# PolarisRisingWar/rgb-experiment

Measured on AMD Instinct MI355X. Metric: aggregated edges/sec (full-graph GCN d=128, reference epoch = train fwd+bwd+Adam + 2 eval fwd), higher is better.
Workload: dtype f32

## Files before the change

include/rgbx_hip.h:

```cpp
#ifndef RGBX_HIP_H
#define RGBX_HIP_H

#include <stddef.h>
#include <stdint.h>

#ifdef __cplusplus
extern "C" {
#endif

#define RGBX_VERSION 501

#define RGBX_OK 0
#define RGBX_E_ARG (-1)
#define RGBX_E_RANGE (-2)
#define RGBX_E_ALIGN (-3)
#define RGBX_E_WS (-4)
#define RGBX_E_SHAPE (-5)

typedef void* rgbx_stream_t;

enum {
  RGBX_LOOPS_KEEP = 0,
  RGBX_LOOPS_ADD_REMAINING = 1,
  RGBX_LOOPS_REMOVE_ADD = 2
// ... 230 lines not shown
int rgbx_masked_nll_bwd_f32(const int64_t* y, const uint8_t* mask, int64_t N, int64_t C,
                            const float* scale, float* grad, int64_t ldg, rgbx_stream_t stream);

int rgbx_masked_ce_fwd_f32(const float* logits, int64_t ld, const int64_t* y, const uint8_t* mask, int64_t N,
                           int64_t C, double* stats, double* scratch, int64_t scratch_doubles,
                           rgbx_stream_t stream);

int rgbx_masked_ce_fwd_blocked_f32(const float* logits, int64_t blk_cols, int64_t blk_stride, const float* bias,
                                   const int64_t* y, const uint8_t* mask, int64_t N, int64_t C, double* stats,
                                   double* scratch, int64_t scratch_doubles, rgbx_stream_t stream);

int rgbx_masked_ce_bwd_f32(const float* logits, int64_t ld, const int64_t* y, const uint8_t* mask, int64_t N,
                           int64_t C, const float* scale, float* grad, int64_t ldg, rgbx_stream_t stream);


int rgbx_coalesce_workspace_bytes(int64_t E, int64_t N, int mirror, size_t* bytes);
int rgbx_coalesce_keys_i64(const int64_t* row, const int64_t* col, int64_t E, int64_t N, int mirror,
                           uint64_t* keys_out, uint64_t* counts, void* workspace, size_t workspace_bytes,
                           rgbx_stream_t stream);
int rgbx_split_edge_keys_i64(const uint64_t* keys, const uint64_t* counts, int64_t cap, int64_t N, int64_t* out_row,
                             int64_t* out_col, rgbx_stream_t stream);

int rgbx_py_random_shuffle_i64(int64_t seed, int64_t n, int64_t* perm);


int rgbx_gather_rows_f32(const float* src, int64_t lds, const int32_t* idx, int64_t n, int64_t d,
                         float* dst, int64_t ldd, rgbx_stream_t stream);

int rgbx_scatter_add_rows_f32(const float* src, int64_t lds, const int32_t* idx, int64_t n,
                              int64_t d, float* dst, int64_t ldd, rgbx_stream_t stream);

int rgbx_paced_copy_f32(const float* src, float* dst, int64_t n, int workgroups, int nontemporal, rgbx_stream_t stream);

#ifdef __cplusplus
}
#endif
#endif
```

rgb_experiment_amd/_lib.py:

```python
import ctypes
import os

import torch

_HERE = os.path.dirname(os.path.abspath(__file__))
LIB_PATH = os.path.join(_HERE, "csrc", "librgbx_hip.so")

_P = ctypes.c_void_p
_I64 = ctypes.c_int64
_I = ctypes.c_int
_F = ctypes.c_float

class RowSplit(ctypes.Structure):
    _fields_ = [("threshold", ctypes.c_int32), ("n_chunks", ctypes.c_int32), ("n_long", ctypes.c_int32),
                ("chunk_begin", ctypes.c_void_p), ("chunk_end", ctypes.c_void_p), ("chunk_row", ctypes.c_void_p),
                ("long_row", ctypes.c_void_p),
                ("long_chunk_ptr", ctypes.c_void_p), ("partial", ctypes.c_void_p)]


class CeEpilogue(ctypes.Structure):
    _fields_ = [("y", ctypes.c_void_p), ("mask", ctypes.c_void_p), ("grad_scale", ctypes.c_void_p),
                ("stats", ctypes.c_void_p), ("scratch", ctypes.c_void_p), ("mask_groups", ctypes.c_int32),
                ("rows", ctypes.c_void_p), ("n_rows", ctypes.c_int64), ("skip_unselected", ctypes.c_int32)]

# ... 21 lines not shown
    "rgbx_inv_degree_f32": [_P, _I64, _P, _P],
    "rgbx_spmm_csr_f32": [_P, _P, _P, _P, _P, _I64, _P, _I64, _P, _P, _I64, _I64, _I64, _F, _F, _P, _P],
    "rgbx_spmm_csr_epilogue_supported": [_I64],
    "rgbx_spmm_csr_epilogue_f32": [_P, _P, _P, _P, _P, _I64, _P, _I64, _P, _P, _I64, _I64, _I64, _F, _F, _P, _P, _P],
    "rgbx_spmm_csr_short_rows_supported": [_I64],
    "rgbx_spmm_csr_short_rows_f32": [_P, _P, _P, _P, _I64, _P, _P, _I64, _I64, _I64, _P],
    "rgbx_spmm_linear_supported": [_I64, _I64, _I],
    "rgbx_spmm_linear_stats_workspace_bytes": [_I64, _I64, ctypes.POINTER(ctypes.c_size_t)],
    "rgbx_spmm_linear_f32": [_P, _P, _P, _P, _P, _I64, _P, _P, _I64, _P, _P, _P, _I64, _P, _I64, _P, _P, _P, _P, _P,
                             ctypes.c_size_t, _P, _I64, _I64, _I64, _P, _P],
    "rgbx_fused_layer_f32": [_P, _P],
    "rgbx_blocked_to_rows_f32": [_P, _I64, _I64, _P, _I64, _I64, _I64, _P, _P],
    "rgbx_appnp_f32": [_P, _P, _P, _P, _I64, _P, _P, _I64, _I64, _I64, _I, _F, _P, _P],
    "rgbx_dagnn_gate_fwd_f32": [_P, _I64, _P, _I64, _I64, _P, _P, _P, _I64, _I64, _I64, _I, _P],
    "rgbx_dagnn_gate_bwd_workspace_bytes": [_I64, ctypes.POINTER(ctypes.c_size_t)],
    "rgbx_dagnn_gate_bwd_f32": [_P, _I64, _P, _I64, _I64, _P, _P, _P, _I64, _P, _I64, _P, _I64, _I64, _P, _P, _P,
                                ctypes.c_size_t, _I64, _I64, _I, _P],
    "rgbx_gru_step_supported": [_I64],
    "rgbx_gru_step_f32": [_P, _P, _P, _I64, _P, _P, _P, _P, _I64, _P, _I64, _P, _I64, _I64, _I64, _P, _P],
    "rgbx_gru_gate_fwd_f32": [_P, _I64, _P, _I64, _P, _I64, _I64, _I64, _P],
    "rgbx_gru_gate_bwd_f32": [_P, _I64, _P, _I64, _P, _I64, _P, _I64, _P, _I64, _I64, _I64, _P],
    "rgbx_gat_scores_f32": [_P, _I64, _P, _P, _P, _P, _I64, _I, _I, _P],
    "rgbx_gat_scores_bwd_scratch_floats": [_I64, _I, _I, ctypes.POINTER(ctypes.c_int64)],
    "rgbx_gat_scores_bwd_f32": [_P, _I64, _P, _P, _I64, _P, _P, _P, _I64, _P, _P, _P, _I64, _I64, _I, _I, _P],
    "rgbx_gat_aggregate_fwd_f32": [_P, _P, _P, _I64, _P, _P, _P, _P, _P, _P, _P, _I64, _P, _P, _P, _P, _I64, _I, _I, _F, _P,
                                   _P],
    "rgbx_gat_edge_softmax_f32": [_P, _P, _P, _P, _F, _P, _P, _P, _P, _P, _I64, _P, _P],
    "rgbx_gat_bwd_dst_f32": [_P, _P, _P, _I64, _P, _P, _P, _P, _P, _I64, _P, _I64, _P, _P, _I64, _I, _I,
                             _F, _P],
    "rgbx_gat_bwd_prep_f32": [_P, _P, _P, _P, _I64, _P, _P, _I64, _P, _P, _P, _F, _P, _I64, _I, _I, _P],
    "rgbx_gat_bwd_src_f32": [_P, _P, _P, _I64, _P, _P, _P, _I64, _P, _I64, _P, _P, _P, _P, _I64, _I, _I, _F, _P, _P],
    "rgbx_gemm_tn_workspace_bytes": [_I64, _I64, _I64, ctypes.POINTER(ctypes.c_size_t)],
    "rgbx_gemm_tn_f32": [_P, _I64, _P, _I64, _P, _I64, _P, _I64, _I64, _I64, _F, _P, ctypes.c_size_t, _P],
    "rgbx_bn_scratch_doubles": [_I64, _I64, ctypes.POINTER(ctypes.c_int64)],
    "rgbx_bn_stats_f32": [_P, _I64, _I64, _I64, _P, _P, _I64, _P],
    "rgbx_bn_finalize_f32": [_P, _P, _P, _F, _F, _P, _P, _P, _P, _P, _P, _I64, _P],
    "rgbx_fold_bn_linear_f32": [_P, _I64, _P, _I64, _P, _P, _P, _P, _P, _P, _F, _P, _P, _P, _I64, _I64, _P],
    "rgbx_bn_bwd_finalize_f32": [_P, _P, _P, _P, _P, _P, _P, _P, _P, _P, _I64, _P],
    "rgbx_affine_cols_f32": [_P, _I64, _P, _P, _P, _I64, _I64, _I64, _P],
    "rgbx_bn_bwd_reduce_f32": [_P, _I64, _P, _I64, _P, _P, _I64, _I64, _P, _P, _I64, _P],
    "rgbx_bn_bwd_apply_f32": [_P, _I64, _P, _I64, _P, _P, _P, _P, _P, _P, _I64, _I64, _I64, _P],
    "rgbx_masked_nll_scratch_doubles": [_I64, _I, ctypes.POINTER(ctypes.c_int64)],
    "rgbx_masked_nll_fwd_f32": [_P, _I64, _P, _P, _I64, _I64, _P, _P, _I64, _I, _P],
    "rgbx_masked_ce_fwd_f32": [_P, _I64, _P, _P, _I64, _I64, _P, _P, _I64, _P],
    "rgbx_masked_ce_fwd_blocked_f32": [_P, _I64, _I64, _P, _P, _P, _I64, _I64, _P, _P, _I64, _P],
    "rgbx_masked_ce_bwd_f32": [_P, _I64, _P, _P, _I64, _I64, _P, _P, _I64, _P],
    "rgbx_masked_nll_bwd_f32": [_P, _P, _I64, _I64, _P, _P, _I64, _P],
    "rgbx_coalesce_workspace_bytes": [_I64, _I64, _I, ctypes.POINTER(ctypes.c_size_t)],
    "rgbx_coalesce_keys_i64": [_P, _P, _I64, _I64, _I, _P, _P, _P, ctypes.c_size_t, _P],
    "rgbx_split_edge_keys_i64": [_P, _P, _I64, _I64, _P, _P, _P],
    "rgbx_gather_rows_f32": [_P, _I64, _P, _I64, _I64, _P, _I64, _P],
    "rgbx_scatter_add_rows_f32": [_P, _I64, _P, _I64, _I64, _P, _I64, _P],
    "rgbx_paced_copy_f32": [_P, _P, _I64, _I, _I, _P],
    "rgbx_py_random_shuffle_i64": [_I64, _I64, _P],
}
EXPORTS = ["rgbx_version", "rgbx_last_error_string"] + list(SIGNATURES)

_lib = None


def bind(path, strict=True):
    lib = ctypes.CDLL(path)
    lib.rgbx_version.restype = _I
    lib.rgbx_version.argtypes = []
    lib.rgbx_last_error_string.restype = ctypes.c_char_p
    lib.rgbx_last_error_string.argtypes = []
# ... 57 lines not shown
```

rgb_experiment_amd/csrc/gemm.hip:

```cpp
#include "rgbx_common.h"

namespace rgbx {
namespace {

constexpr int BM = 128, BN = 128, KT = 32;
using f32x16 = __attribute__((ext_vector_type(16))) float;

template <int W>
__device__ __forceinline__ void stage_tile(float* __restrict__ lds, const float* __restrict__ src,
                                           int64_t ld, int64_t k0, int64_t k_end, int c0, int ncols) {
  const int tid = threadIdx.x;
#pragma unroll 4
  for (int p = 0; p < KT * W / 256; ++p) {
    const int idx = p * 256 + tid;
    const int r = idx / W, c = idx % W;
    const int64_t k = k0 + r;
    lds[r * W + c] = (k < k_end && c0 + c < ncols) ? src[k * ld + c0 + c] : 0.f;
  }
}

template <int W>
__device__ __forceinline__ void fetch_tile(float4 (&regs)[KT * (W / 4) / 256], const float* __restrict__ src, int64_t ld,
                                           int64_t k0, int64_t k_end, int c0, int ncols) {
#pragma unroll
  for (int p = 0; p < KT * (W / 4) / 256; ++p) {
    const int idx = p * 256 + threadIdx.x;
    const int r = idx / (W / 4), c = (idx % (W / 4)) * 4;
    const int64_t k = k0 + r;
    regs[p] = make_float4(0.f, 0.f, 0.f, 0.f);
    if (k < k_end && c0 + c < ncols) regs[p] = *reinterpret_cast<const float4*>(src + k * ld + c0 + c);
  }
}

template <int W>
__device__ __forceinline__ void put_tile(float* __restrict__ lds, const float4 (&regs)[KT * (W / 4) / 256]) {
#pragma unroll
  for (int p = 0; p < KT * (W / 4) / 256; ++p) {
    const int idx = p * 256 + threadIdx.x;
    const int r = idx / (W / 4), c = (idx % (W / 4)) * 4;
    *reinterpret_cast<float4*>(lds + r * W + c) = regs[p];
  }
}

template <bool VEC4, int MT>
__global__ void __launch_bounds__(256)
gemm_tn_partial_kernel(const float* __restrict__ A, int64_t lda, const float* __restrict__ B, int64_t ldb,
                       float* __restrict__ part, float* __restrict__ colpart, int64_t K, int M, int N,
                       int64_t slab) {
  constexpr int MI = MT / 64;
  __shared__ float lds[KT * (MT + 128)];
  float* la = lds;
  float* lb = lds + KT * MT;
  const int split = blockIdx.x;
  const int m0 = blockIdx.y * MT, n0 = blockIdx.z * BN;
  const int64_t k_begin = (int64_t)split * slab;
  const int64_t k_end = k_begin + slab < K ? k_begin + slab : K;
  const int wave = threadIdx.x >> 6, lane = threadIdx.x & 63;
  const int wm = (wave >> 1) * (MT / 2), wn = (wave & 1) * 64;
  const int kr = lane >> 5, cc = lane & 31;

  f32x16 acc[MI][2];
#pragma unroll
  for (int i = 0; i < MI; ++i)
#pragma unroll
    for (int j = 0; j < 2; ++j)
#pragma unroll
      for (int r = 0; r < 16; ++r) acc[i][j][r] = 0.f;

  const bool sums = colpart != nullptr && blockIdx.z == 0 && threadIdx.x < MT;
  float csum = 0.f;
  auto consume = [&]() {
    if (sums) {
#pragma unroll 8
      for (int r = 0; r < KT; ++r) csum += la[r * MT + threadIdx.x];
    }
#pragma unroll 4
    for (int kk = 0; kk < KT; kk += 2) {
      float a[MI];
#pragma unroll
      for (int i = 0; i < MI; ++i) a[i] = la[(kk + kr) * MT + wm + i * 32 + cc];
      const float b0 = lb[(kk + kr) * 128 + wn + cc];
      const float b1 = lb[(kk + kr) * 128 + wn + 32 + cc];
#pragma unroll
      for (int i = 0; i < MI; ++i) {
        acc[i][0] = __builtin_amdgcn_mfma_f32_32x32x2f32(a[i], b0, acc[i][0], 0, 0, 0);
        acc[i][1] = __builtin_amdgcn_mfma_f32_32x32x2f32(a[i], b1, acc[i][1], 0, 0, 0);
      }
    }
  };
  if constexpr (VEC4) {
    float4 ra[KT * (MT / 4) / 256], rb[KT * 32 / 256];
    fetch_tile<MT>(ra, A, lda, k_begin, k_end, m0, M);
    fetch_tile<128>(rb, B, ldb, k_begin, k_end, n0, N);
    for (int64_t k0 = k_begin; k0 < k_end; k0 += KT) {
      __syncthreads();
      put_tile<MT>(la, ra);
      put_tile<128>(lb, rb);
      __syncthreads();
      if (k0 + KT < k_end) {
        fetch_tile<MT>(ra, A, lda, k0 + KT, k_end, m0, M);
        fetch_tile<128>(rb, B, ldb, k0 + KT, k_end, n0, N);
      }
      consume();
    }
  } else {
    for (int64_t k0 = k_begin; k0 < k_end; k0 += KT) {
      __syncthreads();
      stage_tile<MT>(la, A, lda, k0, k_end, m0, M);
      stage_tile<128>(lb, B, ldb, k0, k_end, n0, N);
      __syncthreads();
      consume();
    }
  }

  if (sums && m0 + (int)threadIdx.x < M) colpart[(int64_t)split * M + m0 + threadIdx.x] = csum;
  float* out = part + (int64_t)split * M * N;
#pragma unroll
  for (int i = 0; i < MI; ++i)
#pragma unroll
    for (int j = 0; j < 2; ++j)
#pragma unroll
      for (int r = 0; r < 16; ++r) {
        const int m = m0 + wm + i * 32 + (r & 3) + 8 * (r >> 2) + 4 * kr;
        const int n = n0 + wn + j * 32 + cc;
        if (m < M && n < N) out[(int64_t)m * N + n] = acc[i][j][r];
      }
}

__global__ void __launch_bounds__(256)
gemm_tn_reduce_kernel(const float* __restrict__ part, int S, int64_t MN, float* __restrict__ C, int N,
                      int64_t ldc, float alpha) {
  __shared__ float sh[8][32];
  const int j = threadIdx.x & 31, q = threadIdx.x >> 5;
  for (int64_t base = (int64_t)blockIdx.x * 32; base < MN; base += (int64_t)gridDim.x * 32) {
    const int64_t i = base + j;
    float s = 0.f;
    if (i < MN)
      for (int p = q; p < S; p += 8) s += part[(int64_t)p * MN + i];
    __syncthreads();
    sh[q][j] = s;
    __syncthreads();
    if (q == 0 && i < MN) {
      float t = 0.f;
#pragma unroll
      for (int k = 0; k < 8; ++k) t += sh[k][j];
      C[(i / N) * ldc + (i % N)] = alpha * t;
    }
  }
}

int tile_rows(int M) { return M <= 64 ? 64 : BM; }

int choose_splits(int64_t K, int M, int N) {
  const int64_t tiles = cdiv(M, tile_rows(M)) * cdiv(N, BN);
  int64_t s = cdiv(tile_rows(M) == 64 ? 1024 : 768, tiles);
  const int64_t max_s = cdiv(K, 16 * KT);
  if (s > max_s) s = max_s;
  if (s < 1) s = 1;
  return (int)s;
}

}
}

using namespace rgbx;

extern "C" int rgbx_gemm_tn_workspace_bytes(int64_t K, int64_t M, int64_t N, size_t* bytes) {
  if (!bytes || K < 0 || M < 0 || N < 0) return fail(RGBX_E_ARG, "gemm_tn_workspace_bytes: bad argument");
  if (M >= INT32_MAX || N >= INT32_MAX) return fail(RGBX_E_RANGE, "gemm_tn: M or N exceeds int32");
  *bytes = (size_t)choose_splits(K, (int)M, (int)N) * ((size_t)M * (size_t)N + (size_t)M) * sizeof(float);
  return RGBX_OK;
}

extern "C" int rgbx_gemm_tn_f32(const float* A, int64_t lda, const float* B, int64_t ldb, float* C,
                                int64_t ldc, float* a_colsum, int64_t K, int64_t M, int64_t N, float alpha,
                                void* workspace, size_t workspace_bytes, rgbx_stream_t stream) {
  if (K < 0 || M < 0 || N < 0) return fail(RGBX_E_ARG, "gemm_tn: negative size");
  if (M == 0 || N == 0) return RGBX_OK;
  if (!C || (K > 0 && (!A || !B))) return fail(RGBX_E_ARG, "gemm_tn: null pointer");
  if (M >= INT32_MAX || N >= INT32_MAX) return fail(RGBX_E_RANGE, "gemm_tn: M or N exceeds int32");
  if (lda < M || ldb < N || ldc < N) return fail(RGBX_E_ARG, "gemm_tn: leading dimension too small");
  size_t need = 0;
  if (int rc = rgbx_gemm_tn_workspace_bytes(K, M, N, &need)) return rc;
  if (!workspace || workspace_bytes < need)
    return fail(RGBX_E_WS, "gemm_tn: workspace %zu < %zu bytes", workspace_bytes, need);
  hipStream_t s = (hipStream_t)stream;
  const int S = choose_splits(K, (int)M, (int)N);
  const int64_t slab = cdiv(cdiv(K > 0 ? K : 1, S), KT) * KT;
  float* part = static_cast<float*>(workspace);
  float* colpart = a_colsum ? part + (size_t)S * M * N : nullptr;
  const int mt = tile_rows((int)M);
  dim3 grid(S, (unsigned)cdiv(M, mt), (unsigned)cdiv(N, BN));
  const bool v4 = aligned16(A) && aligned16(B) && lda % 4 == 0 && ldb % 4 == 0;
#define RGBX_GEMM_TN(V4, MT) \
  gemm_tn_partial_kernel<V4, MT><<<grid, 256, 0, s>>>(A, lda, B, ldb, part, colpart, K, (int)M, (int)N, slab)
  if (v4) { if (mt == 64) RGBX_GEMM_TN(true, 64); else RGBX_GEMM_TN(true, 128); }
  else { if (mt == 64) RGBX_GEMM_TN(false, 64); else RGBX_GEMM_TN(false, 128); }
#undef RGBX_GEMM_TN
  RGBX_CHECK_LAUNCH("gemm_tn_partial_kernel");
  const int64_t MN = M * N;
  int64_t rb = cdiv(MN, 32);
  if (rb > kMaxGrid) rb = kMaxGrid;
  gemm_tn_reduce_kernel<<<(int)rb, 256, 0, s>>>(part, S, MN, C, (int)N, ldc, alpha);
  RGBX_CHECK_LAUNCH("gemm_tn_reduce_kernel");
  if (a_colsum) {
    gemm_tn_reduce_kernel<<<(int)cdiv(M, 32), 256, 0, s>>>(colpart, S, M, a_colsum, (int)M, M, 1.0f);
    RGBX_CHECK_LAUNCH("gemm_tn_reduce_kernel");
  }
  return RGBX_OK;
}
```

rgb_experiment_amd/nn/batchnorm.py:

```python
import ctypes

import torch
import torch.nn as nn

from .. import _lib


def _scratch(n, d, device):
    cnt = ctypes.c_int64(0)
    _lib.check(_lib.load().rgbx_bn_scratch_doubles(n, d, ctypes.byref(cnt)), "rgbx_bn_scratch_doubles")
    return torch.empty(cnt.value, dtype=torch.float64, device=device), cnt.value


def column_sums(x):
    if not x.is_cuda:
        xd = x.double()
        return torch.stack([xd.sum(0), (xd * xd).sum(0)])
    px, ldx = _lib.mat(x, "x")
    n, d = x.shape
    sums = torch.empty((2, d), dtype=torch.float64, device=x.device)
    scratch, cnt = _scratch(n, d, x.device)
    _lib.check(_lib.load().rgbx_bn_stats_f32(px, ldx, n, d, _lib.ptr(sums), _lib.ptr(scratch), cnt, _lib.stream_ptr()),
               "rgbx_bn_stats_f32")
    return sums
# ... 59 lines not shown
    sums = colsums if colsums is not None and tuple(colsums.shape) == (2, d) else column_sums(x)
    return torch.cat([sums.reshape(-1), count])


def train_statistics(x, weight, bias, eps, reduce, running, colsums=None, packed=None):
    d = x.size(1)
    if packed is None:
        packed = reduce(pack_statistics(x, colsums))
    n = packed[2 * d:2 * d + 1]
    if x.is_cuda:
        mean, rstd, scale, shift = (torch.empty(d, dtype=torch.float32, device=x.device) for _ in range(4))
        rm, rv, mom = running if running is not None else (None, None, 0.0)
        _lib.check(_lib.load().rgbx_bn_finalize_f32(
            _lib.ptr(packed), _lib.ptr(weight.detach().contiguous()), _lib.ptr(bias.detach().contiguous()),
            float(eps), float(mom), _lib.ptr(rm), _lib.ptr(rv), _lib.ptr(mean), _lib.ptr(rstd), _lib.ptr(scale),
            _lib.ptr(shift), d, _lib.stream_ptr()), "rgbx_bn_finalize_f32")
    else:
        mean64 = packed[:d] / n
        var64 = (packed[d:2 * d] / n - mean64 * mean64).clamp_(min=0.0)
        mean, var = mean64.float(), var64.float()
        rstd = torch.rsqrt(var + eps)
        scale = weight.detach() * rstd
        shift = bias.detach() - mean * scale
        if running is not None:
            rm, rv, mom = running
            unbiased = var * (n / (n - 1).clamp(min=1)).float()
            rm.mul_(1 - mom).add_(mean, alpha=mom)
            rv.mul_(1 - mom).add_(unbiased, alpha=mom)
    return mean, rstd, scale, shift, n


def train_backward(gy, x, weight, mean, rstd, n, reduce, grads_out=None, sums=None):
    gy = gy if gy.stride(-1) == 1 else gy.contiguous()
    d = x.size(1)
    if sums is None:
        local = bwd_sums(gy, x, mean, rstd)
        glob = reduce(local.reshape(-1).clone())
    else:
        local, glob = sums
    if gy.is_cuda:
        ca, cb, ck = (torch.empty(d, dtype=torch.float32, device=gy.device) for _ in range(3))
        gw, gb = grads_out if grads_out is not None else (torch.empty(d, dtype=torch.float32, device=gy.device)
                                                          for _ in range(2))
        _lib.check(_lib.load().rgbx_bn_bwd_finalize_f32(
            _lib.ptr(glob), _lib.ptr(local), _lib.ptr(n), _lib.ptr(weight.detach().contiguous()), _lib.ptr(rstd),
            _lib.ptr(ca), _lib.ptr(cb), _lib.ptr(ck), _lib.ptr(gw), _lib.ptr(gb), d, _lib.stream_ptr()),
            "rgbx_bn_bwd_finalize_f32")
    else:
        glob = glob.reshape(2, -1)
        ca = (glob[0] / n).float().contiguous()
        cb = (glob[1] / n).float().contiguous()
        ck = (weight * rstd).contiguous()
        gw, gb = local[1].float(), local[0].float()
        if grads_out is not None:
            grads_out[0].copy_(gw)
            grads_out[1].copy_(gb)
            gw, gb = grads_out
    return bwd_apply(gy, x, mean, rstd, ca, cb, ck), gw, gb


class _AffineCols(torch.autograd.Function):

    @staticmethod
    def forward(ctx, x, scale, shift):
        x = x if x.stride(-1) == 1 else x.contiguous()
        ctx.save_for_backward(x, scale)
        return affine_cols(x, scale.detach().contiguous(), shift.detach().contiguous())

    @staticmethod
    def backward(ctx, gy):
        x, scale = ctx.saved_tensors
        gy = gy if gy.stride(-1) == 1 else gy.contiguous()
        gx = g_scale = g_shift = None
        if ctx.needs_input_grad[0]:
            gx = affine_cols(gy, scale.detach().contiguous(), torch.zeros_like(scale))
        if ctx.needs_input_grad[1]:
            g_scale = (gy * x).sum(0)
        if ctx.needs_input_grad[2]:
            g_shift = gy.sum(0)
        return gx, g_scale, g_shift


class BatchNorm1d(nn.BatchNorm1d):

    def _reduce(self, packed):
        return packed

    def _reducer(self, x):
        return self._reduce

    def eval_affine(self):
# ... 28 lines not shown
```

rgb_experiment_amd/ops.py:

```python
import ctypes

import torch

from . import _lib

_EVENT_SINK = None


def set_event_sink(sink):
    global _EVENT_SINK
    _EVENT_SINK = sink


class Kind(str):
    variant = None


class _Timed:
    def __init__(self, kind, variant=None):
        if variant is not None and _EVENT_SINK is not None:
            kind = Kind(kind)
            kind.variant = variant
        self.kind = kind

# ... 576 lines not shown
    wrt = torch.empty_like(wt) if Wr is not None else None
    has_b = bias is not None or bias2 is not None or bn is not None
    b_out = torch.empty(n_out, dtype=torch.float32, device=W.device) if has_b else None
    c = lambda t: None if t is None else t.detach().contiguous()
    b1, b2 = c(bias), c(bias2)
    g = be = rm = rv = None
    eps = 0.0
    if bn is not None:
        g, be, rm, rv, eps = c(bn.weight), c(bn.bias), c(bn.running_mean), c(bn.running_var), bn.eps
    _lib.check(_lib.load().rgbx_fold_bn_linear_f32(
        _lib.ptr(W), W.stride(0), _lib.ptr(Wr), 0 if Wr is None else Wr.stride(0), _lib.ptr(b1), _lib.ptr(b2),
        _lib.ptr(g), _lib.ptr(be), _lib.ptr(rm), _lib.ptr(rv), float(eps), _lib.ptr(wt), _lib.ptr(wrt), _lib.ptr(b_out),
        n_out, K, _lib.stream_ptr()), "rgbx_fold_bn_linear_f32")
    return wt, b_out, wrt


class _PropagateLinear(torch.autograd.Function):

    @staticmethod
    def forward(ctx, x, graph, kind, weight, bias, need_z=True, root_weight=None, x_root=None, want_colsums=False):
        x = x.contiguous()
        xr = x if x_root is None else x_root.contiguous()
        w = graph.w if kind == "gcn" else None
        rs = graph.inv_deg if kind == "mean" else None
        if kind not in ("gcn", "mean", "sum"):
            raise ValueError(kind)
        res = spmm_linear_raw(graph.fwd, w, rs, x, weight_t(weight), None if bias is None else bias.detach(),
                              need_z, xr if root_weight is not None else None,
                              None if root_weight is None else weight_t(root_weight),
                              kind=f"{getattr(graph, 'event_prefix', '')}{kind}_linear_fwd", want_colsums=want_colsums)
        out, z = res[0], res[1]
        ctx.save_for_backward(z, weight, root_weight, xr if root_weight is not None else None)
        ctx.graph, ctx.kind, ctx.has_bias = graph, kind, bias is not None
        if want_colsums:
            ctx.mark_non_differentiable(res[2])
            return out, res[2]
        return out

    @staticmethod
    def backward(ctx, gy, _g_colsums=None):
        z, weight, root_weight, x = ctx.saved_tensors
        g, kind = ctx.graph, ctx.kind
        gy = gy.contiguous()
        gx = gw = gb = gwr = None
        want_b = ctx.has_bias and ctx.needs_input_grad[4]
        if ctx.needs_input_grad[3]:
            if want_b:
                gw, gb = gemm_tn(gy, z, colsum=True)
            else:
                gw = gemm_tn(gy, z)
        elif want_b:
            gb = gy.sum(0)
        if root_weight is not None and ctx.needs_input_grad[6]:
            gwr = gemm_tn(gy, x)
        if ctx.needs_input_grad[0]:
            gx = _propagate_linear_input_grad(g, kind, gy, weight, root_weight)
        return gx, None, None, gw, gb, None, gwr, None, None


def _propagate_linear_input_grad(g, kind, gy, weight, root_weight, ce_sel=None):
    csr = g.bwd
    wt = {"gcn": lambda: g.w_t, "mean": lambda: g.w_mean_t, "sum": lambda: None}[kind]()
    prefix = getattr(g, "event_prefix", "")
    n_out, n_in = weight.shape
    if n_out <= n_in and _lib.load().rgbx_spmm_linear_supported(n_out, n_in, int(root_weight is not None)):
        gx, _, _ = fused_layer(gy, weight.detach().contiguous(), csr=csr, w=wt,
                               x_root=gy if root_weight is not None else None,
                               wt_root=None if root_weight is None else root_weight.detach().contiguous(),
                               col_sel=None if ce_sel is None else selected_cols(*ce_sel), kind=f"{prefix}{kind}_linear_bwd")
        return gx
    gz = gy @ weight
    gr = gy @ root_weight if root_weight is not None else None
    if gr is None:
        return spmm_raw(csr, wt, None, gz, kind=f"{prefix}{kind}_bwd")
    return spmm_raw(csr, wt, None, gz, y=gr, a=1.0, b=1.0, out=gr, kind=f"{prefix}{kind}_bwd")


class _BNPropagateLinear(torch.autograd.Function):

    @staticmethod
    def forward(ctx, x, bn_weight, bn_bias, graph, kind, weight, bias, root_weight, eps, reduce, running, need_z,
                colsums=None, want_colsums=False):
        from .nn import batchnorm as B
        x = x.contiguous()
        mean, rstd, scale, shift, n = B.train_statistics(x, bn_weight, bn_bias, eps, reduce, running, colsums)
        w, rs = (graph.w, None) if kind == "gcn" else (None, graph.inv_deg)
        res = spmm_linear_raw(graph.fwd, w, rs, x, weight_t(weight), None if bias is None else bias.detach(), need_z,
                              x if root_weight is not None else None,
                              None if root_weight is None else weight_t(root_weight), kind=f"{kind}_linear_fwd",
                              pre=(scale, shift, graph.rowsum(kind)), want_colsums=want_colsums)
        out, z = res[0], res[1]
        ctx.save_for_backward(x, bn_weight, mean, rstd, n, z, weight, root_weight, scale, shift)
        ctx.graph, ctx.kind, ctx.has_bias, ctx.reduce = graph, kind, bias is not None, reduce
        if want_colsums:
            ctx.mark_non_differentiable(res[2])
            return out, res[2]
        return out

    @staticmethod
    def backward(ctx, gy, _g_colsums=None):
        from .nn import batchnorm as B
        x, bn_weight, mean, rstd, n, z, weight, root_weight, scale, shift = ctx.saved_tensors
        g, kind = ctx.graph, ctx.kind
        gy = gy.contiguous()
        gw = gb = gwr = None
        if ctx.needs_input_grad[5]:
            gw, gcol = gemm_tn(gy, z, colsum=True)
            gb = gcol if ctx.has_bias and ctx.needs_input_grad[6] else None
        else:
            gcol = gy.sum(0)
            gb = gcol if ctx.has_bias and ctx.needs_input_grad[6] else None
        if root_weight is not None and ctx.needs_input_grad[7]:
            gwr = gemm_tn(gy, x) * scale + gcol[:, None] * shift
        g_h = _propagate_linear_input_grad(g, kind, gy, weight, root_weight)
        gx, g_bnw, g_bnb = B.train_backward(g_h, x, bn_weight, mean, rstd, n, ctx.reduce)
        return gx, g_bnw, g_bnb, None, None, gw, gb, gwr, None, None, None, None, None, None


_SCALE_CACHE = {}


def mask_scale(y, mask, C):
    key = (y.data_ptr(), y._version, y.numel(), None if mask is None else (mask.data_ptr(), mask._version), int(C))
    hit = _SCALE_CACHE.get(key)
    if hit is None:
        sel = (y >= 0) & (y < C)
        if mask is not None:
            sel = sel & mask.bool()
        hit = (_MadeOn((1.0 / sel.sum().double()).float().reshape(1)), y, mask)
        _SCALE_CACHE[key] = hit
        while len(_SCALE_CACHE) > 32:
            _SCALE_CACHE.pop(next(iter(_SCALE_CACHE)))
    return hit[0].get()


_GROUP_MASKS = {}


def group_masks(mask_a, mask_b):
    _lib.require_device(mask_a, mask_b)
    key = (mask_a.data_ptr(), mask_a._version, mask_b.data_ptr(), mask_b._version, mask_a.numel())
    hit = _GROUP_MASKS.get(key)
    if hit is None:
        g = (mask_a.bool().to(torch.uint8) | (mask_b.bool().to(torch.uint8) << 1)).contiguous()
        hit = (_MadeOn(g), mask_a, mask_b)
        _GROUP_MASKS[key] = hit
        while len(_GROUP_MASKS) > 16:
            _GROUP_MASKS.pop(next(iter(_GROUP_MASKS)))
# ... 35 lines not shown
def selected_cols(y, mask, C):
    key = _sel_key(y, mask, C)
    hit = _SEL_COLS.get(key)
    if hit is None:
        if torch.cuda.is_current_stream_capturing():
            return None
        hit = (_MadeOn(ce_selection(y, mask, C).to(torch.uint8).contiguous()), y, mask)
        _SEL_COLS[key] = hit
        while len(_SEL_COLS) > 16:
            _SEL_COLS.pop(next(iter(_SEL_COLS)))
    return hit[0].get()



def ce_from_logits(logits, y, mask):
    if isinstance(mask, (tuple, list)):
        return None, torch.stack([masked_ce_accuracy(logits, y, m) for m in mask])
    if torch.is_grad_enabled() and logits.requires_grad:
        return masked_ce_loss(logits, y, mask, with_stats=True)
    stats = masked_ce_accuracy(logits, y, mask)
    return (stats[0] / stats[1]).float(), stats


def fused_ce_ok(graph, in_channels, out_channels, root, x, y):
    return (not _is_dist(graph) and out_channels <= 128 and y is not None and y.is_cuda and y.dtype == torch.int64
            and fused_linear_ok(graph, in_channels, out_channels, root=root, x=x))


class _PropagateLinearCE(torch.autograd.Function):

    @staticmethod
    def forward(ctx, x, graph, kind, weight, bias, root_weight, y, mask, want_grad, bn_weight, bn_bias, bn_args):
        from .nn import batchnorm as B
        x = x.contiguous()
        pre = None
        if bn_weight is not None:
            eps, reduce, running, colsums = bn_args
            mean, rstd, scale, shift, n = B.train_statistics(x, bn_weight, bn_bias, eps, reduce, running, colsums)
            pre = (scale, shift, graph.rowsum(kind))
        w, rs = (graph.w, None) if kind == "gcn" else (None, graph.inv_deg)
        grad_scale = mask_scale(y, mask, weight.size(0)) if want_grad else None
        dlogits, z, stats = spmm_linear_raw(
            graph.fwd, w, rs, x, weight_t(weight), None if bias is None else bias.detach(),
            want_grad and weight.requires_grad, x if root_weight is not None else None,
            None if root_weight is None else weight_t(root_weight), kind=f"{kind}_linear_fwd", pre=pre,
            ce=(y, mask, grad_scale), select_rows=True)
        ctx.graph, ctx.kind, ctx.has_bias, ctx.has_bn = graph, kind, bias is not None, bn_weight is not None
        ctx.ce_sel = (y, mask, weight.size(0)) if want_grad else None
        if want_grad:
            if ctx.has_bn:
                ctx.save_for_backward(dlogits, z, weight, root_weight, x, bn_weight, mean, rstd, n, scale, shift)
                ctx.reduce = bn_args[1]
            else:
                ctx.save_for_backward(dlogits, z, weight, root_weight, x if root_weight is not None else None)
        ctx.mark_non_differentiable(stats)
        if stats.dim() == 2:
            return stats.new_zeros(()).float(), stats
        return (stats[0] / stats[1]).float(), stats

    @staticmethod
    def backward(ctx, g, _g_stats):
        from .nn import batchnorm as B
        saved = ctx.saved_tensors
        if ctx.has_bn:
            gy, z, weight, root_weight, x, bn_weight, mean, rstd, n, scale, shift = saved
        else:
            gy, z, weight, root_weight, x = saved
        graph, kind = ctx.graph, ctx.kind
        g = g.reshape(()).float()
        gw = gb = gwr = gx = g_bnw = g_bnb = None
        gcol = None
        if ctx.needs_input_grad[3]:
            gw, gcol = gemm_tn(gy, z, colsum=True)
        if ctx.has_bias and ctx.needs_input_grad[4]:
            gb = gcol if gcol is not None else gy.sum(0)
        if root_weight is not None and ctx.needs_input_grad[5]:
            if ctx.has_bn:
                gcol = gcol if gcol is not None else gy.sum(0)
                gwr = gemm_tn(gy, x) * scale + gcol[:, None] * shift
            else:
                gwr = gemm_tn(gy, x)
        need_h = ctx.needs_input_grad[0] or (ctx.has_bn and (ctx.needs_input_grad[9] or ctx.needs_input_grad[10]))
        items = [(k, t) for k, t in (("gw", gw), ("gb", gb), ("gwr", gwr)) if t is not None]
        if need_h:
            items.append(("w", weight.detach()))
            if root_weight is not None:
                items.append(("wr", root_weight.detach()))
        sc = dict(zip((k for k, _ in items), torch._foreach_mul([t for _, t in items], g))) if items else {}
        gw, gb, gwr = sc.get("gw"), sc.get("gb"), sc.get("gwr")
        if need_h:
            g_h = _propagate_linear_input_grad(graph, kind, gy, sc["w"], sc.get("wr"), ce_sel=ctx.ce_sel)
            if ctx.has_bn:
                gx, g_bnw, g_bnb = B.train_backward(g_h, x, bn_weight, mean, rstd, n, ctx.reduce)
            else:
                gx = g_h
        return gx, None, None, gw, gb, gwr, None, None, None, g_bnw, g_bnb, None


def propagate_linear_ce(x, graph, kind, weight, bias, root_weight, y, mask, bn=None, colsums=None):
    want_grad = not isinstance(mask, (tuple, list)) and torch.is_grad_enabled() and any(
        t is not None and t.requires_grad
        for t in (weight, x, bias, root_weight) + ((bn.weight, bn.bias) if bn is not None else ()))
    if bn is not None:
        bn_args = (bn.eps, bn._reduce, bn.begin_training_step(), colsums)
        return _PropagateLinearCE.apply(x, graph, kind, weight, bias, root_weight, y, mask, want_grad, bn.weight, bn.bias,
                                        bn_args)
    return _PropagateLinearCE.apply(x, graph, kind, weight, bias, root_weight, y, mask, want_grad, None, None, None)


def bn_propagate_linear(x, bn, graph, kind, weight, bias=None, root_weight=None, colsums=None, want_colsums=False):
    need_z = weight.requires_grad
    return _tag_colsums(_BNPropagateLinear.apply(x, bn.weight, bn.bias, graph, kind, weight, bias, root_weight, bn.eps,
                                                 bn._reduce, bn.begin_training_step(), need_z, colsums, want_colsums),
                        want_colsums)


COLSUMS = "_rgbx_colsums"


def _tag_colsums(res, want_colsums):
    if not want_colsums:
        return res
    out, colsums = res
    setattr(out, COLSUMS, colsums)
    return out

# ... 647 lines not shown
                                              _lib.stream_ptr()), "rgbx_scatter_add_rows_f32")
    return dst



def gemm_tn(a, b, alpha=1.0, colsum=False, out=None, sums_out=None):
    _lib.require_device(a, b)
    a = a if a.stride(-1) == 1 and _rows_padded_readable(a) else a.contiguous()
    b = b if b.stride(-1) == 1 and _rows_padded_readable(b) else b.contiguous()
    if a.size(0) >= 4096:
        a, b = (_aligned_rows(t) for t in (a, b))
    pa, lda = _lib.mat(a, "a")
    pb, ldb = _lib.mat(b, "b")
    K, M, N = a.size(0), a.size(1), b.size(1)
    lib = _lib.load()
    nbytes = ctypes.c_size_t(0)
    _lib.check(lib.rgbx_gemm_tn_workspace_bytes(K, M, N, ctypes.byref(nbytes)), "rgbx_gemm_tn_workspace_bytes")
    ws = torch.empty(max(nbytes.value, 1), dtype=torch.uint8, device=a.device)
    if out is None:
        out = torch.empty((M, N), dtype=torch.float32, device=a.device)
    elif tuple(out.shape) != (M, N) or not out.is_contiguous() or out.dtype != torch.float32:
        raise RuntimeError(f"gemm_tn: out must be a contiguous float32 [{M}, {N}] tensor")
    sums = None
    if colsum:
        sums = sums_out if sums_out is not None else torch.empty(M, dtype=torch.float32, device=a.device)
        if tuple(sums.shape) != (M,) or not sums.is_contiguous() or sums.dtype != torch.float32:
            raise RuntimeError(f"gemm_tn: sums_out must be a contiguous float32 [{M}] tensor")
    with _Timed("gemm_tn", f"{M}x{N}" if _EVENT_SINK is not None else None):
        _lib.check(lib.rgbx_gemm_tn_f32(pa, lda, pb, ldb, _lib.ptr(out), N, _lib.ptr(sums), K, M, N, float(alpha),
                                        _lib.ptr(ws), ws.numel(), _lib.stream_ptr()), "rgbx_gemm_tn_f32")
    return (out, sums) if colsum else out


class _Linear(torch.autograd.Function):

    @staticmethod
    def forward(ctx, x, weight, bias):
        ctx.save_for_backward(x, weight)
        ctx.has_bias = bias is not None
        if _EVENT_SINK is None or not x.is_cuda:
            return torch.nn.functional.linear(x, weight, bias)
        with _Timed("linear_fwd", f"{weight.size(1)}->{weight.size(0)}"):
            return torch.nn.functional.linear(x, weight, bias)

    @staticmethod
    def backward(ctx, gy):
        x, weight = ctx.saved_tensors
        gy = gy.contiguous()
        gx = gy @ weight if ctx.needs_input_grad[0] else None
        gw = gb = None
        want_b = ctx.has_bias and ctx.needs_input_grad[2]
        if ctx.needs_input_grad[1] and gy.is_cuda and want_b:
            gw, gb = gemm_tn(gy, x, colsum=True)
        else:
            if ctx.needs_input_grad[1]:
                gw = gemm_tn(gy, x) if gy.is_cuda else gy.t() @ x
            gb = gy.sum(0) if want_b else None
        return gx, gw, gb


def linear(x, weight, bias=None):
    sp = getattr(x, "_rgbx_sparse", None)
    if sp is not None and not x.requires_grad:
        return _SparseRowsLinear.apply(sp, weight, bias)
    return _Linear.apply(x, weight, bias)

# ... 254 lines not shown
```

Baseline: 16.51 billion.

## Fuse BatchNorm backward apply into producer layer's weight-gradient GEMM

Adds a gemm_tn variant that applies the BatchNorm input-gradient transform (using x, mean, rstd and per-column coefficients) on the fly while staging the A tile. The BN backward hands its coefficients to the producing propagate-linear node instead of materialising the BN input gradient, and that node computes its weight and bias gradients directly from the fused GEMM. This removes one full N×d elementwise pass and its write and read-back, at the cost of extra loads of x inside the GEMM and some autograd plumbing (materialize_grads off, handoff through ctx).

Result: slower. 16.30 billion (median of 2 runs) (-1.3%).

```diff
diff --git a/include/rgbx_hip.h b/include/rgbx_hip.h
--- a/include/rgbx_hip.h
+++ b/include/rgbx_hip.h
@@ -286,6 +286,12 @@
 
 int rgbx_paced_copy_f32(const float* src, float* dst, int64_t n, int workgroups, int nontemporal, rgbx_stream_t stream);
 
+
+int rgbx_gemm_tn_bn_f32(const float* gy, int64_t ldg, const float* x, int64_t ldx, const float* mean, const float* rstd,
+                        const float* ca, const float* cb, const float* ck, const float* B, int64_t ldb, float* C,
+                        int64_t ldc, float* a_colsum, int64_t K, int64_t M, int64_t N, float alpha, void* workspace,
+                        size_t workspace_bytes, rgbx_stream_t stream);
+
 #ifdef __cplusplus
 }
 #endif
diff --git a/rgb_experiment_amd/_lib.py b/rgb_experiment_amd/_lib.py
--- a/rgb_experiment_amd/_lib.py
+++ b/rgb_experiment_amd/_lib.py
@@ -77,6 +77,8 @@
     "rgbx_gat_bwd_src_f32": [_P, _P, _P, _I64, _P, _P, _P, _I64, _P, _I64, _P, _P, _P, _P, _I64, _I, _I, _F, _P, _P],
     "rgbx_gemm_tn_workspace_bytes": [_I64, _I64, _I64, ctypes.POINTER(ctypes.c_size_t)],
     "rgbx_gemm_tn_f32": [_P, _I64, _P, _I64, _P, _I64, _P, _I64, _I64, _I64, _F, _P, ctypes.c_size_t, _P],
+    "rgbx_gemm_tn_bn_f32": [_P, _I64, _P, _I64, _P, _P, _P, _P, _P, _P, _I64, _P, _I64, _P, _I64, _I64, _I64, _F, _P,
+                            ctypes.c_size_t, _P],
     "rgbx_bn_scratch_doubles": [_I64, _I64, ctypes.POINTER(ctypes.c_int64)],
     "rgbx_bn_stats_f32": [_P, _I64, _I64, _I64, _P, _P, _I64, _P],
     "rgbx_bn_finalize_f32": [_P, _P, _P, _F, _F, _P, _P, _P, _P, _P, _P, _I64, _P],
diff --git a/rgb_experiment_amd/csrc/gemm.hip b/rgb_experiment_amd/csrc/gemm.hip
--- a/rgb_experiment_amd/csrc/gemm.hip
+++ b/rgb_experiment_amd/csrc/gemm.hip
@@ -5,6 +5,16 @@
 
 constexpr int BM = 128, BN = 128, KT = 32;
 using f32x16 = __attribute__((ext_vector_type(16))) float;
+
+struct BnBwdMap {
+  const float* x;
+  int64_t ldx;
+  const float *mean, *rstd, *ca, *cb, *ck;
+};
+
+__device__ __forceinline__ float bn_bwd_elem(float g, float v, float mu, float rs, float a, float b, float k) {
+  return fmaf(-((v - mu) * rs), b, g - a) * k;
+}
 
 template <int W>
 __device__ __forceinline__ void stage_tile(float* __restrict__ lds, const float* __restrict__ src,
@@ -20,6 +30,22 @@
 }
 
 template <int W>
+__device__ __forceinline__ void stage_tile_bn(float* __restrict__ lds, const float* __restrict__ src, int64_t ld,
+                                              const BnBwdMap& bn, int64_t k0, int64_t k_end, int c0, int ncols) {
+  const int tid = threadIdx.x;
+#pragma unroll 4
+  for (int p = 0; p < KT * W / 256; ++p) {
+    const int idx = p * 256 + tid;
+    const int r = idx / W, c = idx % W, m = c0 + c;
+    const int64_t k = k0 + r;
+    lds[r * W + c] = (k < k_end && m < ncols)
+                         ? bn_bwd_elem(src[k * ld + m], bn.x[k * bn.ldx + m], bn.mean[m], bn.rstd[m], bn.ca[m], bn.cb[m],
+                                       bn.ck[m])
+                         : 0.f;
+  }
+}
+
+template <int W>
 __device__ __forceinline__ void fetch_tile(float4 (&regs)[KT * (W / 4) / 256], const float* __restrict__ src, int64_t ld,
                                            int64_t k0, int64_t k_end, int c0, int ncols) {
 #pragma unroll
@@ -42,15 +68,34 @@
   }
 }
 
-template <bool VEC4, int MT>
+template <int W>
+__device__ __forceinline__ void map_tile_bn(float4 (&g)[KT * (W / 4) / 256], const float4 (&v)[KT * (W / 4) / 256],
+                                            const float* __restrict__ cst, int64_t k0, int64_t k_end, int c0, int ncols) {
+  const int c = (threadIdx.x % (W / 4)) * 4;
+#pragma unroll
+  for (int j = 0; j < 4; ++j) {
+    const float mu = cst[0 * W + c + j], rs = cst[1 * W + c + j], ca = cst[2 * W + c + j], cb = cst[3 * W + c + j],
+                ck = cst[4 * W + c + j];
+#pragma unroll
+    for (int p = 0; p < KT * (W / 4) / 256; ++p) {
+      const int r = (p * 256 + threadIdx.x) / (W / 4);
+      float* gp = reinterpret_cast<float*>(&g[p]);
+      const float* vp = reinterpret_cast<const float*>(&v[p]);
+      gp[j] = (k0 + r < k_end && c0 + c < ncols) ? bn_bwd_elem(gp[j], vp[j], mu, rs, ca, cb, ck) : 0.f;
+    }
+  }
+}
+
+template <bool VEC4, int MT, bool BNA>
 __global__ void __launch_bounds__(256)
 gemm_tn_partial_kernel(const float* __restrict__ A, int64_t lda, const float* __restrict__ B, int64_t ldb,
                        float* __restrict__ part, float* __restrict__ colpart, int64_t K, int M, int N,
-                       int64_t slab) {
+                       int64_t slab, BnBwdMap bn) {
   constexpr int MI = MT / 64;
-  __shared__ float lds[KT * (MT + 128)];
+  __shared__ float lds[KT * (MT + 128) + (BNA ? 5 * MT : 0)];
   float* la = lds;
   float* lb = lds + KT * MT;
+  float* lc = lds + KT * (MT + 128);
   const int split = blockIdx.x;
   const int m0 = blockIdx.y * MT, n0 = blockIdx.z * BN;
   const int64_t k_begin = (int64_t)split * slab;
@@ -58,6 +103,13 @@
   const int wave = threadIdx.x >> 6, lane = threadIdx.x & 63;
   const int wm = (wave >> 1) * (MT / 2), wn = (wave & 1) * 64;
   const int kr = lane >> 5, cc = lane & 31;
+  if constexpr (BNA && VEC4) {
+    for (int i = threadIdx.x; i < 5 * MT; i += 256) {
+      const int m = m0 + i % MT;
+      const float* src = i < MT ? bn.mean : i < 2 * MT ? bn.rstd : i < 3 * MT ? bn.ca : i < 4 * MT ? bn.cb : bn.ck;
+      lc[i] = m < M ? src[m] : 0.f;
+    }
+  }
 
   f32x16 acc[MI][2];
 #pragma unroll
@@ -89,16 +141,20 @@
     }
   };
   if constexpr (VEC4) {
-    float4 ra[KT * (MT / 4) / 256], rb[KT * 32 / 256];
+    constexpr int NX = BNA ? KT * (MT / 4) / 256 : 0;
+    float4 ra[KT * (MT / 4) / 256], rb[KT * 32 / 256], rx[NX > 0 ? NX : 1];
     fetch_tile<MT>(ra, A, lda, k_begin, k_end, m0, M);
+    if constexpr (BNA) fetch_tile<MT>(rx, bn.x, bn.ldx, k_begin, k_end, m0, M);
     fetch_tile<128>(rb, B, ldb, k_begin, k_end, n0, N);
     for (int64_t k0 = k_begin; k0 < k_end; k0 += KT) {
       __syncthreads();
+      if constexpr (BNA) map_tile_bn<MT>(ra, rx, lc, k0, k_end, m0, M);
       put_tile<MT>(la, ra);
       put_tile<128>(lb, rb);
       __syncthreads();
       if (k0 + KT < k_end) {
         fetch_tile<MT>(ra, A, lda, k0 + KT, k_end, m0, M);
+        if constexpr (BNA) fetch_tile<MT>(rx, bn.x, bn.ldx, k0 + KT, k_end, m0, M);
         fetch_tile<128>(rb, B, ldb, k0 + KT, k_end, n0, N);
       }
       consume();
@@ -106,7 +162,8 @@
   } else {
     for (int64_t k0 = k_begin; k0 < k_end; k0 += KT) {
       __syncthreads();
-      stage_tile<MT>(la, A, lda, k0, k_end, m0, M);
+      if constexpr (BNA) stage_tile_bn<MT>(la, A, lda, bn, k0, k_end, m0, M);
+      else stage_tile<MT>(la, A, lda, k0, k_end, m0, M);
       stage_tile<128>(lb, B, ldb, k0, k_end, n0, N);
       __syncthreads();
       consume();
@@ -172,30 +229,30 @@
   return RGBX_OK;
 }
 
-extern "C" int rgbx_gemm_tn_f32(const float* A, int64_t lda, const float* B, int64_t ldb, float* C,
-                                int64_t ldc, float* a_colsum, int64_t K, int64_t M, int64_t N, float alpha,
-                                void* workspace, size_t workspace_bytes, rgbx_stream_t stream) {
-  if (K < 0 || M < 0 || N < 0) return fail(RGBX_E_ARG, "gemm_tn: negative size");
-  if (M == 0 || N == 0) return RGBX_OK;
-  if (!C || (K > 0 && (!A || !B))) return fail(RGBX_E_ARG, "gemm_tn: null pointer");
-  if (M >= INT32_MAX || N >= INT32_MAX) return fail(RGBX_E_RANGE, "gemm_tn: M or N exceeds int32");
-  if (lda < M || ldb < N || ldc < N) return fail(RGBX_E_ARG, "gemm_tn: leading dimension too small");
-  size_t need = 0;
-  if (int rc = rgbx_gemm_tn_workspace_bytes(K, M, N, &need)) return rc;
-  if (!workspace || workspace_bytes < need)
-    return fail(RGBX_E_WS, "gemm_tn: workspace %zu < %zu bytes", workspace_bytes, need);
-  hipStream_t s = (hipStream_t)stream;
+namespace rgbx {
+namespace {
+
+int run_gemm_tn(const float* A, int64_t lda, const float* B, int64_t ldb, float* C, int64_t ldc, float* a_colsum,
+                int64_t K, int64_t M, int64_t N, float alpha, void* workspace, size_t workspace_bytes, hipStream_t s,
+                const BnBwdMap* bn) {
   const int S = choose_splits(K, (int)M, (int)N);
   const int64_t slab = cdiv(cdiv(K > 0 ? K : 1, S), KT) * KT;
   float* part = static_cast<float*>(workspace);
   float* colpart = a_colsum ? part + (size_t)S * M * N : nullptr;
   const int mt = tile_rows((int)M);
   dim3 grid(S, (unsigned)cdiv(M, mt), (unsigned)cdiv(N, BN));
-  const bool v4 = aligned16(A) && aligned16(B) && lda % 4 == 0 && ldb % 4 == 0;
-#define RGBX_GEMM_TN(V4, MT) \
-  gemm_tn_partial_kernel<V4, MT><<<grid, 256, 0, s>>>(A, lda, B, ldb, part, colpart, K, (int)M, (int)N, slab)
-  if (v4) { if (mt == 64) RGBX_GEMM_TN(true, 64); else RGBX_GEMM_TN(true, 128); }
-  else { if (mt == 64) RGBX_GEMM_TN(false, 64); else RGBX_GEMM_TN(false, 128); }
+  bool v4 = aligned16(A) && aligned16(B) && lda % 4 == 0 && ldb % 4 == 0;
+  if (bn) v4 = v4 && aligned16(bn->x) && bn->ldx % 4 == 0;
+  const BnBwdMap map = bn ? *bn : BnBwdMap{};
+#define RGBX_GEMM_TN(V4, MT, BNA) \
+  gemm_tn_partial_kernel<V4, MT, BNA><<<grid, 256, 0, s>>>(A, lda, B, ldb, part, colpart, K, (int)M, (int)N, slab, map)
+  if (!bn) {
+    if (v4) { if (mt == 64) RGBX_GEMM_TN(true, 64, false); else RGBX_GEMM_TN(true, 128, false); }
+    else { if (mt == 64) RGBX_GEMM_TN(false, 64, false); else RGBX_GEMM_TN(false, 128, false); }
+  } else {
+    if (v4) { if (mt == 64) RGBX_GEMM_TN(true, 64, true); else RGBX_GEMM_TN(true, 128, true); }
+    else { if (mt == 64) RGBX_GEMM_TN(false, 64, true); else RGBX_GEMM_TN(false, 128, true); }
+  }
 #undef RGBX_GEMM_TN
   RGBX_CHECK_LAUNCH("gemm_tn_partial_kernel");
   const int64_t MN = M * N;
@@ -209,3 +266,43 @@
   }
   return RGBX_OK;
 }
+
+int check_gemm_tn(const char* name, const float* A, int64_t lda, const float* B, int64_t ldb, float* C, int64_t ldc,
+                  int64_t K, int64_t M, int64_t N, void* workspace, size_t workspace_bytes) {
+  if (K < 0 || M < 0 || N < 0) return fail(RGBX_E_ARG, "%s: negative size", name);
+  if (M == 0 || N == 0) return RGBX_OK;
+  if (!C || (K > 0 && (!A || !B))) return fail(RGBX_E_ARG, "%s: null pointer", name);
+  if (M >= INT32_MAX || N >= INT32_MAX) return fail(RGBX_E_RANGE, "%s: M or N exceeds int32", name);
+  if (lda < M || ldb < N || ldc < N) return fail(RGBX_E_ARG, "%s: leading dimension too small", name);
+  size_t need = 0;
+  if (int rc = rgbx_gemm_tn_workspace_bytes(K, M, N, &need)) return rc;
+  if (!workspace || workspace_bytes < need)
+    return fail(RGBX_E_WS, "%s: workspace %zu < %zu bytes", name, workspace_bytes, need);
+  return RGBX_OK;
+}
+
+}
+}
+
+extern "C" int rgbx_gemm_tn_f32(const float* A, int64_t lda, const float* B, int64_t ldb, float* C,
+                                int64_t ldc, float* a_colsum, int64_t K, int64_t M, int64_t N, float alpha,
+                                void* workspace, size_t workspace_bytes, rgbx_stream_t stream) {
+  if (int rc = check_gemm_tn("gemm_tn", A, lda, B, ldb, C, ldc, K, M, N, workspace, workspace_bytes)) return rc;
+  if (M == 0 || N == 0) return RGBX_OK;
+  return run_gemm_tn(A, lda, B, ldb, C, ldc, a_colsum, K, M, N, alpha, workspace, workspace_bytes,
+                     (hipStream_t)stream, nullptr);
+}
+
+extern "C" int rgbx_gemm_tn_bn_f32(const float* gy, int64_t ldg, const float* x, int64_t ldx, const float* mean,
+                                   const float* rstd, const float* ca, const float* cb, const float* ck, const float* B,
+                                   int64_t ldb, float* C, int64_t ldc, float* a_colsum, int64_t K, int64_t M, int64_t N,
+                                   float alpha, void* workspace, size_t workspace_bytes, rgbx_stream_t stream) {
+  if (int rc = check_gemm_tn("gemm_tn_bn", gy, ldg, B, ldb, C, ldc, K, M, N, workspace, workspace_bytes)) return rc;
+  if (M == 0 || N == 0) return RGBX_OK;
+  if (K > 0 && (!x || !mean || !rstd || !ca || !cb || !ck))
+    return fail(RGBX_E_ARG, "gemm_tn_bn: null pointer");
+  if (ldx < M) return fail(RGBX_E_ARG, "gemm_tn_bn: leading dimension too small");
+  const BnBwdMap bn{x, ldx, mean, rstd, ca, cb, ck};
+  return run_gemm_tn(gy, ldg, B, ldb, C, ldc, a_colsum, K, M, N, alpha, workspace, workspace_bytes, (hipStream_t)stream,
+                     &bn);
+}
diff --git a/rgb_experiment_amd/nn/batchnorm.py b/rgb_experiment_amd/nn/batchnorm.py
--- a/rgb_experiment_amd/nn/batchnorm.py
+++ b/rgb_experiment_amd/nn/batchnorm.py
@@ -115,6 +115,11 @@
 
 def train_backward(gy, x, weight, mean, rstd, n, reduce, grads_out=None, sums=None):
     gy = gy if gy.stride(-1) == 1 else gy.contiguous()
+    ca, cb, ck, gw, gb = train_backward_coeffs(gy, x, weight, mean, rstd, n, reduce, grads_out, sums)
+    return bwd_apply(gy, x, mean, rstd, ca, cb, ck), gw, gb
+
+
+def train_backward_coeffs(gy, x, weight, mean, rstd, n, reduce, grads_out=None, sums=None):
     d = x.size(1)
     if sums is None:
         local = bwd_sums(gy, x, mean, rstd)
@@ -139,7 +144,11 @@
             grads_out[0].copy_(gw)
             grads_out[1].copy_(gb)
             gw, gb = grads_out
-    return bwd_apply(gy, x, mean, rstd, ca, cb, ck), gw, gb
+    return ca, cb, ck, gw, gb
+
+
+def identity_reduce(reduce):
+    return getattr(reduce, "__func__", None) is BatchNorm1d._reduce
 
 
 class _AffineCols(torch.autograd.Function):
diff --git a/rgb_experiment_amd/ops.py b/rgb_experiment_amd/ops.py
--- a/rgb_experiment_amd/ops.py
+++ b/rgb_experiment_amd/ops.py
@@ -632,6 +632,8 @@
         out, z = res[0], res[1]
         ctx.save_for_backward(z, weight, root_weight, xr if root_weight is not None else None)
         ctx.graph, ctx.kind, ctx.has_bias = graph, kind, bias is not None
+        ctx.set_materialize_grads(False)
+        ctx.out_shape = tuple(out.shape)
         if want_colsums:
             ctx.mark_non_differentiable(res[2])
             return out, res[2]
@@ -641,9 +643,24 @@
     def backward(ctx, gy, _g_colsums=None):
         z, weight, root_weight, x = ctx.saved_tensors
         g, kind = ctx.graph, ctx.kind
-        gy = gy.contiguous()
+        hand, ctx.bn_handoff = getattr(ctx, "bn_handoff", None), None
         gx = gw = gb = gwr = None
         want_b = ctx.has_bias and ctx.needs_input_grad[4]
+        if hand is not None and gy is None and ctx.needs_input_grad[3] and not ctx.needs_input_grad[0]:
+            if want_b:
+                gw, gb = gemm_tn_bn(*hand, z, colsum=True)
+            else:
+                gw = gemm_tn_bn(*hand, z)
+            if root_weight is not None and ctx.needs_input_grad[6]:
+                gwr = gemm_tn_bn(*hand, x)
+            return None, None, None, gw, gb, None, gwr, None, None
+        if hand is not None:
+            from .nn import batchnorm as B
+            dy = B.bwd_apply(*hand)
+            gy = dy if gy is None else gy + dy
+        elif gy is None:
+            gy = torch.zeros(ctx.out_shape, dtype=torch.float32, device=weight.device)
+        gy = gy.contiguous()
         if ctx.needs_input_grad[3]:
             if want_b:
                 gw, gb = gemm_tn(gy, z, colsum=True)
@@ -676,12 +693,35 @@
     return spmm_raw(csr, wt, None, gz, y=gr, a=1.0, b=1.0, out=gr, kind=f"{prefix}{kind}_bwd")
 
 
+FUSE_BN_BACKWARD = True
+
+
+def _bn_producer(x):
+    fn = x.grad_fn
+    if isinstance(fn, _PropagateLinear._backward_cls) and not fn.needs_input_grad[0]:
+        return fn
+    return None
+
+
+def _bn_backward(ctx, g_h, x, bn_weight, mean, rstd, n):
+    from .nn import batchnorm as B
+    prod = getattr(ctx, "bn_producer", None)
+    if (prod is not None and FUSE_BN_BACKWARD and g_h.is_cuda and B.identity_reduce(ctx.reduce) and x.size(1) % 4 == 0
+            and x.is_contiguous()):
+        g_h = g_h if g_h.is_contiguous() else g_h.contiguous()
+        ca, cb, ck, g_bnw, g_bnb = B.train_backward_coeffs(g_h, x, bn_weight, mean, rstd, n, ctx.reduce)
+        prod.bn_handoff = (g_h, x, mean, rstd, ca, cb, ck)
+        return None, g_bnw, g_bnb
+    return B.train_backward(g_h, x, bn_weight, mean, rstd, n, ctx.reduce)
+
+
 class _BNPropagateLinear(torch.autograd.Function):
 
     @staticmethod
     def forward(ctx, x, bn_weight, bn_bias, graph, kind, weight, bias, root_weight, eps, reduce, running, need_z,
                 colsums=None, want_colsums=False):
         from .nn import batchnorm as B
+        ctx.bn_producer = _bn_producer(x)
         x = x.contiguous()
         mean, rstd, scale, shift, n = B.train_statistics(x, bn_weight, bn_bias, eps, reduce, running, colsums)
         w, rs = (graph.w, None) if kind == "gcn" else (None, graph.inv_deg)
@@ -699,7 +739,6 @@
 
     @staticmethod
     def backward(ctx, gy, _g_colsums=None):
-        from .nn import batchnorm as B
         x, bn_weight, mean, rstd, n, z, weight, root_weight, scale, shift = ctx.saved_tensors
         g, kind = ctx.graph, ctx.kind
         gy = gy.contiguous()
@@ -713,7 +752,7 @@
         if root_weight is not None and ctx.needs_input_grad[7]:
             gwr = gemm_tn(gy, x) * scale + gcol[:, None] * shift
         g_h = _propagate_linear_input_grad(g, kind, gy, weight, root_weight)
-        gx, g_bnw, g_bnb = B.train_backward(g_h, x, bn_weight, mean, rstd, n, ctx.reduce)
+        gx, g_bnw, g_bnb = _bn_backward(ctx, g_h, x, bn_weight, mean, rstd, n)
         return gx, g_bnw, g_bnb, None, None, gw, gb, gwr, None, None, None, None, None, None
 
 
@@ -815,6 +854,7 @@
     @staticmethod
     def forward(ctx, x, graph, kind, weight, bias, root_weight, y, mask, want_grad, bn_weight, bn_bias, bn_args):
         from .nn import batchnorm as B
+        ctx.bn_producer = _bn_producer(x) if bn_weight is not None else None
         x = x.contiguous()
         pre = None
         if bn_weight is not None:
@@ -843,7 +883,6 @@
 
     @staticmethod
     def backward(ctx, g, _g_stats):
-        from .nn import batchnorm as B
         saved = ctx.saved_tensors
         if ctx.has_bn:
             gy, z, weight, root_weight, x, bn_weight, mean, rstd, n, scale, shift = saved
@@ -874,7 +913,7 @@
         if need_h:
             g_h = _propagate_linear_input_grad(graph, kind, gy, sc["w"], sc.get("wr"), ce_sel=ctx.ce_sel)
             if ctx.has_bn:
-                gx, g_bnw, g_bnb = B.train_backward(g_h, x, bn_weight, mean, rstd, n, ctx.reduce)
+                gx, g_bnw, g_bnb = _bn_backward(ctx, g_h, x, bn_weight, mean, rstd, n)
             else:
                 gx = g_h
         return gx, None, None, gw, gb, gwr, None, None, None, g_bnw, g_bnb, None
@@ -1588,6 +1627,28 @@
     return (out, sums) if colsum else out
 
 
+def gemm_tn_bn(gy, x, mean, rstd, ca, cb, ck, b, colsum=False):
+    _lib.require_device(gy, x, b)
+    b = b if b.stride(-1) == 1 and _rows_padded_readable(b) else b.contiguous()
+    if b.size(0) >= 4096:
+        b = _aligned_rows(b)
+    pg, ldg = _lib.mat(gy, "gy")
+    px, ldx = _lib.mat(x, "x")
+    pb, ldb = _lib.mat(b, "b")
+    K, M, N = gy.size(0), gy.size(1), b.size(1)
+    lib = _lib.load()
+    nbytes = ctypes.c_size_t(0)
+    _lib.check(lib.rgbx_gemm_tn_workspace_bytes(K, M, N, ctypes.byref(nbytes)), "rgbx_gemm_tn_workspace_bytes")
+    ws = torch.empty(max(nbytes.value, 1), dtype=torch.uint8, device=gy.device)
+    out = torch.empty((M, N), dtype=torch.float32, device=gy.device)
+    sums = torch.empty(M, dtype=torch.float32, device=gy.device) if colsum else None
+    with _Timed("gemm_tn_bn", f"{M}x{N}" if _EVENT_SINK is not None else None):
+        _lib.check(lib.rgbx_gemm_tn_bn_f32(pg, ldg, px, ldx, _lib.ptr(mean), _lib.ptr(rstd), _lib.ptr(ca), _lib.ptr(cb),
+                                           _lib.ptr(ck), pb, ldb, _lib.ptr(out), N, _lib.ptr(sums), K, M, N, 1.0,
+                                           _lib.ptr(ws), ws.numel(), _lib.stream_ptr()), "rgbx_gemm_tn_bn_f32")
+    return (out, sums) if colsum else out
+
+
 class _Linear(torch.autograd.Function):
 
     @staticmethod
```
